# AI4quantum/qiskit-gym

Hardware: AMD Instinct MI355X
Metric: env-steps/sec (whole node), CliffordGym 16q x 65536 envs/GPU; bit-exact vs CPU (higher is better)
Workload: dtype u32

## Files before the change

### qiskit_gym_amd/csrc/kernels_qm_step1.hip

```cpp
#include "device_common.hpp"
#include "qgym_plan.hpp"
#include "qm_step1.hpp"

namespace qg {

constexpr uint32_t QM_STEP1_BLOCK = 256;

template <int NXP, bool HAS_Z, bool FEAT, bool LIST = false, bool DENSE = false>
__global__ __launch_bounds__(QM_STEP1_BLOCK) void qm_step1_kernel(const void *actions, int32_t *depth, uint32_t *bad, const GateEntry *gates, void *state,
                                                                   uint64_t B, uint32_t flags, uint32_t num_actions, StepArgs a) {
    KernelClock kclk(a.kclk, a.kclk_waves, QM_STEP1_BLOCK);
    constexpr int R = HAS_Z ? 2 * NXP : NXP, G = R / 4;
    constexpr int D16 = DENSE ? R / 16 : 0;
    const Step1Front f{actions, depth, bad, gates, state, B, flags, num_actions};
    const uint64_t env = (uint64_t)blockIdx.x * QM_STEP1_BLOCK + threadIdx.x;
    const uint64_t wave_envs = __builtin_amdgcn_ballot_w64(env < B);
    if constexpr (LIST) {
        bool fin = false;
        if (env < B) fin = qm_step1_mask_body<HAS_Z, FEAT, D16>(f, a, G, env, wave_envs);
        done_mask_store(a.done_mask, B, fin, env, a.done_epoch);
    } else {
        if (env >= B) return;
        (void)qm_step1_mask_body<HAS_Z, FEAT, D16>(f, a, G, env, wave_envs);
    }
}

template <int NXP, bool HAS_Z>
static hipError_t launch_step1(const StepArgs &a, hipStream_t s) {
    const dim3 grid((unsigned)((a.B + QM_STEP1_BLOCK - 1) / QM_STEP1_BLOCK)), block(QM_STEP1_BLOCK);
    const bool feat = a.flags & (F_TRACK | F_LAYERS);
    const bool list = a.flags & F_DONE_LIST;
#define QM_STEP1_LAUNCH(...) \
    hipLaunchKernelGGL((qm_step1_kernel<NXP, HAS_Z, __VA_ARGS__>), grid, block, 0, s, a.actions, a.depth, a.bad, a.gates, a.state, a.B, a.flags, a.num_actions, a)
    constexpr int R = HAS_Z ? 2 * NXP : NXP;
    if constexpr (R % 16 == 0) {
        if (a.dense) {
            if (feat && list) QM_STEP1_LAUNCH(true, true, true);
            else if (feat) QM_STEP1_LAUNCH(true, false, true);
            else if (list) QM_STEP1_LAUNCH(false, true, true);
            else QM_STEP1_LAUNCH(false, false, true);
            return hipGetLastError();
        }
    }
    if (feat && list) QM_STEP1_LAUNCH(true, true);
    else if (feat) QM_STEP1_LAUNCH(true);
    else if (list) QM_STEP1_LAUNCH(false, true);
    else QM_STEP1_LAUNCH(false);
#undef QM_STEP1_LAUNCH
    return hipGetLastError();
}

hipError_t qm_step1(const StepArgs &a, uint32_t nxp, bool has_z, hipStream_t s) {
    if (!a.B) return hipSuccess;
    if (has_z) {
        switch (nxp) {
        case 4: return launch_step1<4, true>(a, s);
        case 8: return launch_step1<8, true>(a, s);
        case 12: return launch_step1<12, true>(a, s);
        case 16: return launch_step1<16, true>(a, s);
        }
    } else {
        switch (nxp) {
        case 4: return launch_step1<4, false>(a, s);
        case 8: return launch_step1<8, false>(a, s);
        case 12: return launch_step1<12, false>(a, s);
        case 16: return launch_step1<16, false>(a, s);
        case 20: return launch_step1<20, false>(a, s);
        case 24: return launch_step1<24, false>(a, s);
        case 28: return launch_step1<28, false>(a, s);
        case 32: return launch_step1<32, false>(a, s);
        }
    }
    return hipErrorInvalidValue;
}

}
```

### qiskit_gym_amd/csrc/qgym_api.cpp

```cpp
#include <atomic>
#include <hip/hip_runtime.h>

#include <algorithm>
#include <cmath>
#include <cctype>
#include <cstdarg>
#include <cstdio>
#include <cstdlib>
#include <cstring>
#include <memory>
#include <string>
#include <vector>

#include "pauli_common.hpp"

namespace qg {

static thread_local std::string g_err;

int set_error(int code, const char *fmt, ...) {
    char buf[512];
    va_list ap;
    va_start(ap, fmt);
    vsnprintf(buf, sizeof buf, fmt, ap);
// ... 213 lines not shown
    static const char *one_q[] = {"h", "s", "sdg", "sx", "sxdg"};
    static const char *two_q[] = {"cx", "cz", "swap"};
    for (int k = 0; k < 5; ++k)
        if (key == one_q[k]) {
            if (n != 1) return set_error(QG_ERR_INVALID, "Gate `%s` expects 1 index, got %zu", name.c_str(), n);
            out->kind = k;
            out->q0 = (int32_t)idx[0];
            out->q1 = 0;
            return QG_OK;
        }
    for (int k = 0; k < 3; ++k)
        if (key == two_q[k]) {
            if (n != 2) return set_error(QG_ERR_INVALID, "Gate `%s` expects 2 indices, got %zu", name.c_str(), n);
            out->kind = 5 + k;
            out->q0 = (int32_t)idx[0];
            out->q1 = (int32_t)idx[1];
            return QG_OK;
        }
    return set_error(QG_ERR_INVALID, "Unknown gate name `%s`. Allowed: H, S, Sdg, SX, SXdg, CX, CZ, SWAP", name.c_str());
}


static int vec_free_buffers(qg_vec *v) {
    void *ptrs[] = {v->state, v->own_depth ? v->depth : nullptr, v->own_reward ? v->reward : nullptr,
                    v->own_done ? v->done : nullptr, v->own_success ? v->success : nullptr, v->inverted, v->own_error ? v->error : nullptr, v->sol,
                    v->sol_len, v->layers, v->d_gates, v->d_descs, v->scratch, v->d_prog,
                    v->d_qubit_perms, v->d_act_perms, v->perm_idx, v->d_gen_tables, v->d_nonsymp, v->bad, v->done_list, v->done_list_alt, v->done_list_spare, v->done_mask[0], v->done_mask[1], v->mask_count, v->d_rowops, v->embed_dump, v->host_in, v->host_obs, v->fault_scratch, v->d_twist_obs, v->twist_words};
    for (void *p : ptrs)
        if (p) (void)hipFree(p);
    drop_graphs(v);
    if (v->capture_stream) (void)hipStreamDestroy(v->capture_stream);
    if (v->fault_word) (void)hipHostFree(v->fault_word);
    if (v->count_seen) (void)hipHostFree(v->count_seen);
    return 0;
}

static int drop_done_list(qg_vec *v, hipStream_t s) { return zero_list_length(v, v->done_list, v->dl.drop(), s); }

static void fill_init_args(const qg_vec *v, InitArgs &a) {
    memset(&a, 0, sizeof a);
    a.tree_grid = plan::tree_grid(v->B);
    a.state = v->state;
    a.depth = v->depth;
    a.reward = v->reward;
    a.done = v->done;
    a.success = v->success;
    a.inverted = v->inverted;
    a.error = v->error;
    a.sol_len = v->sol_len;
    a.layers = v->layers;
    a.layers_len = v->layers_len;
    a.gates = v->d_gates;
    a.B = v->B;
    a.D = v->plan.D;
    a.N = v->N;
    a.num_actions = (uint32_t)v->gates.size();
    a.clock = v->clock_dev;
    a.env_base = v->env_base;
    a.bad = v->bad;
    a.rowops = v->d_rowops;
    a.inverts = (v->plan.flags & F_INVERTS) ? 1u : 0u;
    a.check_symplectic = (plan::is_tile(v->plan) && (v->plan.flags & F_INVERTS)) ? 1u : 0u;
}

static hipError_t launch_init(const qg_vec *v, const InitArgs &a_in, hipStream_t s) {
    InitArgs a = a_in;
    a.kclk = kernel_clock_slot(v);
    a.kclk_waves = v->kclk_waves;
    switch (v->plan.layout) {
    case LAYOUT_LFD: return lfd_init(a, v->plan.w64, v->plan.nxp, v->d_descs, s);
    case LAYOUT_LF8: return lf8_init(a, s);
    case LAYOUT_PERM: return perm_init(a, s);
    case LAYOUT_PERMB: return permb_init(a, v->plan.nxp, v->d_descs, s);
    case LAYOUT_TILE: return qm_init(a, v->plan.nxp, v->plan.has_z, s);
    case LAYOUT_TILE64: return q64_init(a, v->plan.nxp, v->plan.has_z, s);
    default: return hipErrorInvalidValue;
    }
}

static hipError_t launch_step(const qg_vec *v, const StepArgs &a_in, hipStream_t s) {
    StepArgs a = a_in;
    a.kclk = kernel_clock_slot(v);
    a.kclk_waves = v->kclk_waves;
    switch (v->plan.layout) {
    case LAYOUT_LFD: return lfd_step(a, v->plan.w64, v->plan.nxp, s);
    case LAYOUT_LF8: return lf8_step(a, a.T > 1, s);
    case LAYOUT_PERM: return perm_step(a, a.T > 1, s);
    case LAYOUT_PERMB: return permb_step(a, v->plan.nxp, s);
    case LAYOUT_PAULI: return pauli_step(v, a, s);
    case LAYOUT_TILE: return qm_step(a, v->plan.nxp, v->plan.has_z, s);
    case LAYOUT_TILE64: return q64_step(a, v->plan.nxp, v->plan.has_z, s);
    default: return hipErrorInvalidValue;
    }
}

static bool dense_rides_in_step(const qg_vec *v) {
    return v->dense && plan::dense_in_kernel(v->plan, plan::step_kernel_of(v->plan, 1, false, false, v->maybe_nonsymplectic, (uint32_t)v->gates.size(), false));
}

int qg_vec_create(const qg_config *cfg, const qg_gate *gates, size_t n_gates, uint64_t batch, int device, qg_vec **out) {
    if (!cfg || !out || (!gates && n_gates)) return set_error(QG_ERR_INVALID, "null argument");
    *out = nullptr;
    if (cfg->num_qubits <= 0) return set_error(QG_ERR_INVALID, "num_qubits must be positive");
    if (cfg->max_depth < 0 || cfg->depth_slope < 0 || cfg->difficulty < 0)
        return set_error(QG_ERR_INVALID, "difficulty, depth_slope and max_depth are usize in the reference");
    if (batch == 0) return set_error(QG_ERR_INVALID, "batch must be positive");
    const uint32_t N = (uint32_t)cfg->num_qubits;
    for (size_t i = 0; i < n_gates; ++i) {
        const qg_gate &g = gates[i];
        if (g.kind < 0 || g.kind > QG_SWAP) return set_error(QG_ERR_INVALID, "gate %zu: unknown kind %d", i, g.kind);
        bool two = g.kind >= QG_CX;
        if (g.q0 < 0 || (uint32_t)g.q0 >= N || (two && (g.q1 < 0 || (uint32_t)g.q1 >= N)))
            return set_error(QG_ERR_INVALID, "gate %zu: qubit index out of range for %u qubits", i, N);
    }

    int ndev = qg_device_count();
    if (ndev <= 0) return set_error(QG_ERR_DEVICE, "no HIP device visible: libqgym has no CPU fallback");
    if (device < 0 || device >= ndev) return set_error(QG_ERR_INVALID, "device %d out of range (%d visible)", device, ndev);
    qg::DeviceGuard guard(device);
    if (guard.err != hipSuccess) {
        (void)hipGetLastError();
        return set_error(QG_ERR_DEVICE, "cannot select device %d: %s", device, hipGetErrorString(guard.err));
    }
    hipDeviceProp_t prop;
    HIP_TRY(hipGetDeviceProperties(&prop, device));
    if (strncmp(prop.gcnArchName, "gfx950", 6) != 0)
        return set_error(QG_ERR_DEVICE, "device %d is %s; libqgym is built for gfx950 (MI355X) only", device, prop.gcnArchName);

    std::unique_ptr<qg_vec> v(new qg_vec());
    v->cfg = *cfg;
    v->gates.assign(gates, gates + n_gates);
    v->B = batch;
    v->N = N;
    v->device = device;
    v->difficulty = cfg->difficulty;
    v->coin_seed = 0x5EED0000C01Full;

    const char *why = "";
    if (int rc = plan::handle_plan(*cfg, batch, v->plan, why)) return set_error(rc, "%s (num_qubits = %u)", why, N);
    const plan::HandlePlan &hp = v->plan;
    if (hp.layout == LAYOUT_PAULI) v->cfg.max_rotations = hp.max_rotations;
    const bool layers = hp.flags & F_LAYERS;

    std::vector<GateEntry> table(std::max<size_t>(n_gates, 1));
    std::vector<uint32_t> descs(std::max<size_t>(n_gates, 1));
    const float w[4] = {cfg->w_n_cnots, cfg->w_n_layers_cnots, cfg->w_n_layers, cfg->w_n_gates};
    for (size_t i = 0; i < n_gates; ++i) {
        int dc, dg;
        gate_deltas(gates[i], N, dc, dg);
        table[i].ops = cfg->env_kind == QG_PAULI ? 0u
                       : hp.layout == LAYOUT_TILE ? tile_ops(cfg->env_kind, gates[i], false)
                       : hp.layout == LAYOUT_TILE64 ? tile_ops(cfg->env_kind, gates[i], true)
                                                  : gate_ops(cfg->env_kind, gates[i], N);
        table[i].penalty = table_penalty(w, dc, dg);
        descs[i] = make_desc((uint32_t)gates[i].kind, (uint32_t)gates[i].q0, (uint32_t)gates[i].q1);
    }

    qg_vec *p = v.get();
    auto fail = [&](int rc) {
        vec_free_buffers(p);
        return rc;
    };
#define HIP_TRY_V(expr)                                                                            \
    do {                                                                                           \
        hipError_t _e = (expr);                                                                    \
        if (_e != hipSuccess) {                                                                    \
// ... 1022 lines not shown
```

### qiskit_gym_amd/csrc/qgym_internal.hpp

```cpp
#pragma once

#include <hip/hip_runtime.h>
#include <stdint.h>

#include "../../include/qgym.h"

namespace qg {

struct GateEntry {
    uint32_t ops;
    float penalty;
};
static_assert(sizeof(GateEntry) == 8, "GateEntry must be 8 bytes");

enum : uint32_t { OP_NONE = 0, OP_XOR = 1, OP_SWAP = 2 };
__host__ __device__ inline uint32_t make_op(uint32_t type, uint32_t dst, uint32_t src) {
    return (dst & 63u) | ((src & 63u) << 6) | ((type & 3u) << 12);
}

__host__ __device__ inline uint32_t make_desc(uint32_t kind, uint32_t q0, uint32_t q1) {
    return (kind & 0xFFu) | ((q0 & 0xFFu) << 8) | ((q1 & 0xFFu) << 16);
}

enum : uint32_t {
    F_ACT64 = 1u << 0,
    F_INVERTS = 1u << 1,
    F_TRACK = 1u << 2,
    F_LAYERS = 1u << 3,
    F_GJ = 1u << 4,
    F_DONE_LIST = 1u << 5,
    F_GROUP_LANES = 1u << 6
};

__host__ __device__ inline uint64_t done_mask_words(uint64_t B) { return 4ull * ((B + 255ull) / 256ull); }
__host__ __device__ inline uint64_t done_mask_bytes(uint64_t B) { return done_mask_words(B) * 10ull + 8ull; }

__host__ __device__ inline uint64_t splitmix64(uint64_t x) {
    x += 0x9E3779B97F4A7C15ull;
    x = (x ^ (x >> 30)) * 0xBF58476D1CE4E5B9ull;
    x = (x ^ (x >> 27)) * 0x94D049BB133111EBull;
    return x ^ (x >> 31);
}
__host__ __device__ inline uint64_t rng_draw(uint64_t seed, uint64_t env, uint64_t t) {
    return splitmix64(seed ^ splitmix64(env * 0x9E3779B97F4A7C15ull + t));
}
__host__ __device__ inline uint32_t rng_action(uint64_t seed, uint64_t env, uint64_t t, uint32_t num_actions) {
#if defined(__HIP_DEVICE_COMPILE__)
    return (uint32_t)__umul64hi(rng_draw(seed, env, t), (uint64_t)num_actions);
#else
    return (uint32_t)(((unsigned __int128)rng_draw(seed, env, t) * (unsigned __int128)num_actions) >> 64);
#endif
}

struct StepArgs {
    void *state;
    const void *actions;
    const uint8_t *coins;
    const GateEntry *gates;
    const uint32_t *descs;
    int32_t *depth;
    float *reward;
    uint8_t *done;
    uint8_t *success;
    uint8_t *inverted;
    uint32_t *error;
    uint32_t *sol;
    int32_t *sol_len;
    int32_t *layers;
    float *rewards_seq;
    uint8_t *dones_seq;
    uint64_t B;
    uint64_t seed;
    uint64_t step_index;
    uint32_t D;
    uint32_t N;
    uint32_t log2L;
    uint32_t num_actions;
    uint32_t T;
    uint32_t flags;
    uint32_t sol_cap;
    float w[4];
    float pauli_layer_reward;
    uint32_t max_rotations;
    uint32_t kclk_waves;
    const uint64_t *clock;
    uint64_t env_base;
    uint32_t *bad;
    unsigned long long *kclk;
    uint32_t *done_list;
    uint32_t *done_count;
    int8_t *dense;
    uint64_t *done_mask;
    uint32_t done_epoch;
};

#if defined(__HIP_DEVICE_COMPILE__) && !defined(QG_NO_ARG_PREFETCH)
#define QG_PREFETCH_STEP_ARGS(a)                                                                                                          \
    asm volatile("" ::"s"((a).state), "s"((a).actions), "s"((a).gates), "s"((a).depth), "s"((a).bad), "s"((a).B), "s"((a).flags),        \
                 "s"((a).num_actions), "s"((a).N), "s"((a).rewards_seq), "s"((a).dones_seq), "s"((a).reward), "s"((a).done), "s"((a).success), \
                 "s"((a).kclk))
#else
#define QG_PREFETCH_STEP_ARGS(a) ((void)0)
#endif

constexpr uint64_t QG_COMPACT_MIN_ENVS = 4096;
constexpr uint64_t QG_STREAM_MIN_ENVS = 64;

struct InitArgs {
    void *state;
    int32_t *depth;
    float *reward;
    uint8_t *done;
    uint8_t *success;
    uint8_t *inverted;
// ... 123 lines not shown
```

### qiskit_gym_amd/csrc/qgym_plan.hpp

```cpp
#pragma once

#include <stdint.h>
#include <stdio.h>

#include "qgym_internal.hpp"

namespace qg {

enum Layout { LAYOUT_NONE = 0, LAYOUT_LF8 = 2, LAYOUT_PERM = 3, LAYOUT_PAULI = 4, LAYOUT_TILE = 5, LAYOUT_TILE64 = 6, LAYOUT_PERMB = 7, LAYOUT_LFD = 8 };

namespace plan {

constexpr uint32_t MAX_PERMUTATION_QUBITS = 256;
constexpr uint32_t MAX_LINEAR_FUNCTION_QUBITS = 64;
constexpr uint32_t MAX_CLIFFORD_QUBITS = 32;
constexpr uint32_t MAX_PAULI_QUBITS = 32;
constexpr uint32_t MAX_PAULI_ROTATIONS = 32;

struct HandlePlan {
    Layout layout = LAYOUT_NONE;
    uint32_t D = 0;
    uint32_t nxp = 0;
    bool has_z = false;
    bool w64 = false;
// ... 74 lines not shown
    if (p.layout == LAYOUT_NONE && p.D <= 32) {
        p.layout = LAYOUT_TILE;
        p.nxp = (N + 3u) & ~3u;
        p.has_z = cfg.env_kind == QG_CLIFFORD;
        p.state_bytes = ((batch + 63) / 64) * (size_t)row_slots(p) * 256;
    }
    if (p.layout == LAYOUT_NONE) {
        p.layout = LAYOUT_TILE64;
        p.has_z = cfg.env_kind == QG_CLIFFORD;
        p.nxp = p.has_z ? 2u * ((N + 3u) & ~3u) : ((N + 7u) & ~7u);
        p.state_bytes = ((batch + 63) / 64) * (size_t)p.nxp * 512;
    }
    if (inverts) p.flags |= F_INVERTS;
    if (cfg.track_solution) p.flags |= F_TRACK;
    if (!(cfg.w_n_layers == 0.0f && cfg.w_n_layers_cnots == 0.0f)) p.flags |= F_LAYERS;
    p.has_bad = (is_tile(p) && !(p.flags & F_INVERTS)) || p.layout == LAYOUT_PERMB || p.layout == LAYOUT_LFD;
    p.has_done_list = is_tile(p) || p.layout == LAYOUT_PAULI;
    if (!p.state_bytes) p.state_bytes = p.stride_bytes * batch;
    return QG_OK;
}

struct CopyRegion {
    uint32_t offset;
    uint32_t rows;
    uint32_t w;
};
constexpr uint32_t COPY_MAX_STATE_REGIONS = 3;
struct CopyLayout {
    CopyRegion r[COPY_MAX_STATE_REGIONS];
    uint32_t n = 0;
    uint32_t tile_bytes = 0;
};
inline CopyLayout copy_layout(const HandlePlan &p) {
    CopyLayout c;
    auto add = [&c](uint32_t rows, uint32_t w) {
        c.r[c.n++] = CopyRegion{c.tile_bytes, rows, w};
        c.tile_bytes += rows * 64u * w;
    };
    switch (p.layout) {
    case LAYOUT_TILE: add(row_slots(p) / 4u, 16); break;
    case LAYOUT_TILE64: add(row_slots(p) / 2u, 16); break;
    case LAYOUT_PERMB: add(p.nxp, 16); break;
    case LAYOUT_LFD: add(2 * p.nxp, 16); break;
    case LAYOUT_LF8:
    case LAYOUT_PERM: add(1, 8); break;
    case LAYOUT_PAULI: {
        const uint32_t meta = p.pt_rm > 16 ? 3u : 1u;
        if (p.pauli_compact) {
            add(p.pt_nq, 12);
            add(p.pt_rm, 8);
            add(meta, 16);
        } else {
            add(p.pt_nq + p.pt_rm + meta, 16);
        }
        break;
    }
    default: break;
    }
    return c;
}
inline void copy_kernel_name(const HandlePlan &p, char *out, size_t cap) {
    const CopyLayout c = copy_layout(p);
    int at = snprintf(out, cap, "copy_envs_kernel [");
    for (uint32_t i = 0; i < c.n && at >= 0 && (size_t)at < cap; ++i)
        at += snprintf(out + at, cap - (size_t)at, "%s%ux%u", i ? " " : "", c.r[i].rows, c.r[i].w);
    if (at >= 0 && (size_t)at < cap) snprintf(out + at, cap - (size_t)at, "]");
}

constexpr uint32_t tile_group_shift(bool has_z) { return has_z ? 1u : 2u; }
constexpr uint32_t GROUP_LANES_MAX_ACTIONS = 256, GROUP_TABLE_DWORDS = 64;
constexpr uint32_t tile_group_byte(uint32_t ops, bool has_z) {
    return ((ops & 31u) >> tile_group_shift(has_z)) | ((((ops >> 5) & 31u) >> tile_group_shift(has_z)) << 4);
}
inline void gate_group_bytes(const uint32_t *ops, size_t stride, size_t num_actions, bool has_z, uint32_t *out) {
    for (uint32_t j = 0; j < GROUP_TABLE_DWORDS; ++j) out[j] = 0;
    for (size_t i = 0; i < num_actions && i < GROUP_LANES_MAX_ACTIONS; ++i) out[i >> 2] |= tile_group_byte(ops[i * stride], has_z) << (8u * (i & 3u));
}

constexpr uint64_t GROUP_LANES_ENVS_PER_WORKGROUP = 256;
constexpr uint64_t GROUP_LANES_WORKGROUPS_PER_CU = 3;
inline bool group_lanes_pays(Layout layout, size_t num_actions, uint64_t batch, uint32_t compute_units) {
    return layout == LAYOUT_TILE && num_actions <= GROUP_LANES_MAX_ACTIONS &&
           batch <= GROUP_LANES_WORKGROUPS_PER_CU * GROUP_LANES_ENVS_PER_WORKGROUP * compute_units;
}

enum StepKernel {
    SK_INVALID = 0,
    SK_QM_STEP1,
    SK_QM_INV2,
    SK_QM_STEP_INV,
    SK_QM_STEP_GJ,
    SK_QM_FUSED_LDS,
    SK_QM_STEP,
    SK_Q64_STEP1, SK_Q64_INV2, SK_Q64_STEP_INV, SK_Q64_STEP_GJ, SK_Q64_FUSED_LDS, SK_Q64_STEP,
    SK_LFD_STEP,
    SK_WORD_STEP,
    SK_PERMB_STEP1, SK_PERMB_STEP,
    SK_PTILE_STEP1C, SK_PTILE_STEP1, SK_PTILE_FUSED1C, SK_PTILE_STEP,
};
inline const char *step_kernel_name(StepKernel k) {
    switch (k) {
    case SK_QM_STEP1: return "qm_step1_kernel";
    case SK_QM_INV2: return "qm_inv2_kernel";
    case SK_QM_STEP_INV: return "qm_step_kernel<inv>";
    case SK_QM_STEP_GJ: return "qm_step_kernel<gauss-jordan>";
    case SK_QM_FUSED_LDS: return "qm_fused_lds_kernel";
    case SK_QM_STEP: return "qm_step_kernel";
    case SK_Q64_STEP1: return "q64_step1_kernel";
    case SK_Q64_INV2: return "q64_inv2_kernel";
    case SK_Q64_STEP_INV: return "q64_step_kernel<inv>";
    case SK_Q64_STEP_GJ: return "q64_step_kernel<gauss-jordan>";
    case SK_Q64_FUSED_LDS: return "q64_fused_lds_kernel";
    case SK_Q64_STEP: return "q64_step_kernel";
    case SK_LFD_STEP: return "lfd_step_kernel";
    case SK_WORD_STEP: return "word_step_kernel";
    case SK_PERMB_STEP1: return "permb_step1_kernel";
    case SK_PERMB_STEP: return "permb_step_kernel";
    case SK_PTILE_STEP1C: return "ptile_step1c_kernel";
    case SK_PTILE_STEP1: return "ptile_step1_kernel";
    case SK_PTILE_FUSED1C: return "ptile_fused1c_kernel";
    case SK_PTILE_STEP: return "ptile_step_kernel";
    default: return "(none)";
    }
}

inline StepKernel tile_step(bool wide, bool inv_kernels, uint32_t flags, uint32_t T, bool has_bad, bool seq_outputs, uint32_t num_actions) {
    const bool feat = flags & (F_TRACK | F_LAYERS);
    const bool seq = T != 1 || seq_outputs;
    if (has_bad && T == 1 && !(flags & F_INVERTS)) return wide ? SK_Q64_STEP1 : SK_QM_STEP1;
    if (flags & F_INVERTS) {
        if (!inv_kernels) return SK_INVALID;
        if (!(flags & F_GJ) && T == 1) return wide ? SK_Q64_INV2 : SK_QM_INV2;
        if (flags & F_GJ) return wide ? SK_Q64_STEP_GJ : SK_QM_STEP_GJ;
        return wide ? SK_Q64_STEP_INV : SK_QM_STEP_INV;
    }
    if (!feat && seq && T > 1 && num_actions != 0) return wide ? SK_Q64_FUSED_LDS : SK_QM_FUSED_LDS;
    return wide ? SK_Q64_STEP : SK_QM_STEP;
}
constexpr bool tile_inv_kernels(bool wide, bool has_z, uint32_t nxp) { return has_z && (wide || nxp <= 16); }
inline StepKernel permb_step_kernel_of(uint32_t flags, uint32_t T, bool has_bad) {
    return (T == 1 && !(flags & F_INVERTS) && has_bad) ? SK_PERMB_STEP1 : SK_PERMB_STEP;
}
inline StepKernel pauli_step_kernel_of(uint32_t flags, uint32_t T, bool compact, bool has_perms) {
    const bool feat = flags & (F_TRACK | F_LAYERS);
    if (T == 1) return compact ? SK_PTILE_STEP1C : SK_PTILE_STEP1;
    if (!feat && !has_perms && compact) return SK_PTILE_FUSED1C;
    return SK_PTILE_STEP;
}
inline StepKernel step_kernel_of(const HandlePlan &p, uint32_t T, bool fused, bool seq_outputs, bool maybe_nonsymplectic, uint32_t num_actions, bool has_perms) {
    const uint32_t flags = p.flags | (maybe_nonsymplectic ? F_GJ : 0u);
    const uint32_t launch_T = fused ? T : 1u;
    switch (p.layout) {
    case LAYOUT_TILE:
    case LAYOUT_TILE64: {
        const bool wide = p.layout == LAYOUT_TILE64;
        return tile_step(wide, tile_inv_kernels(wide, p.has_z, p.nxp), flags, launch_T, p.has_bad, seq_outputs, num_actions);
    }
    case LAYOUT_LFD: return SK_LFD_STEP;
    case LAYOUT_LF8:
    case LAYOUT_PERM: return SK_WORD_STEP;
    case LAYOUT_PERMB: return permb_step_kernel_of(flags, launch_T, p.has_bad);
    case LAYOUT_PAULI: return pauli_step_kernel_of(flags, launch_T, p.pauli_compact, has_perms);
    default: return SK_INVALID;
    }
}
inline bool step_leaves_done_list(const HandlePlan &p, uint64_t batch, bool maybe_nonsymplectic) {
// ... 69 lines not shown
```

### qiskit_gym_amd/csrc/qm_step1.hpp

```cpp
#pragma once

#include "device_common.hpp"

namespace qg {

#define QM_IDENTITY 0x8421u

template <bool HAS_Z>
__device__ inline void qm_group_get(const uint32_t (&u)[4], uint32_t q, uint32_t &x, uint32_t &z) {
    const uint32_t o = 0u - (q & 1u);
    if constexpr (HAS_Z) {
        x = (u[2] & o) | (u[0] & ~o);
        z = (u[3] & o) | (u[1] & ~o);
    } else {
        const uint32_t h = 0u - ((q >> 1) & 1u);
        const uint32_t lo = (u[1] & o) | (u[0] & ~o), hi = (u[3] & o) | (u[2] & ~o);
        x = (hi & h) | (lo & ~h);
        z = 0u;
    }
}
template <bool HAS_Z>
__device__ inline void qm_group_put(uint32_t (&u)[4], uint32_t q, uint32_t x, uint32_t z) {
    if constexpr (HAS_Z) {
        const uint32_t o = 0u - (q & 1u);
// ... 149 lines not shown
    if (layered) lt = layers_begin(layer_rec(a.layers, env, 2 * a.N + 2), a.N, a.descs[act]);
    const uint32_t ops = g.ops, q0 = ops & 31u, q1 = (ops >> 5) & 31u;
    GateMasks<HAS_Z> gm(ops, g0, g1);
    uint32_t e0[4], e1[4];
#pragma unroll
    for (uint32_t k = 0; k < 4; ++k) {
        e0[k] = HAS_Z ? gm.o0 : 0u - (uint32_t)((q0 & 3u) == k);
        e1[k] = HAS_Z ? gm.o1 : 0u - (uint32_t)((q1 & 3u) == k);
    }
    const uint32_t live = 0u - (uint32_t)(((ops >> 10) & 0xFFFFu) != QM_IDENTITY);
    const uint32_t zb = 1u << a.N;
    uint32_t ix0 = 1u << q0, ix1 = 1u << q1, iz0 = zb << q0, iz1 = zb << q1;
    uint32_t set0 = live & 1u, set1 = set0 & (uint32_t)(q0 != q1);
    uint32_t bad_rest = bad0 & ~((set0 << q0) | (set1 << q1));
    r_solved = 1.0f - penalty; r_open = 0.0f - penalty;
    fin_open = (uint32_t)(depth == 0);
    const bool apart = g0 != g1;
    gm.pin();
    if constexpr (!HAS_Z) asm volatile("" : "+v"(e0[0]), "+v"(e0[1]), "+v"(e0[2]), "+v"(e0[3]), "+v"(e1[0]), "+v"(e1[1]), "+v"(e1[2]), "+v"(e1[3]));
    asm volatile("" : "+v"(ix0), "+v"(ix1), "+v"(iz0), "+v"(iz1), "+v"(set0), "+v"(set1), "+v"(bad_rest), "+v"(r_solved), "+v"(r_open),
                      "+v"(depth), "+v"(fin_open));
    __builtin_amdgcn_sched_barrier(0);
    uint32_t z0, z1;
    const uint32_t x0 = gm.get(ua, gm.o0, gm.h0, z0), x1 = gm.get(ub, gm.o1, gm.h1, z1);
    const uint32_t nx0 = gm.mix(0, x0, z0, x1, z1), nx1 = gm.mix(2, x0, z0, x1, z1);
    const uint32_t nz0 = HAS_Z ? gm.mix(1, x0, z0, x1, z1) : 0u, nz1 = HAS_Z ? gm.mix(3, x0, z0, x1, z1) : 0u;
    gate_put<HAS_Z>(ub, e1, nx1, nz1);
    ua.x = bit_select(gm.same, ub.x, ua.x); ua.y = bit_select(gm.same, ub.y, ua.y);
    ua.z = bit_select(gm.same, ub.z, ua.z); ua.w = bit_select(gm.same, ub.w, ua.w);
    gate_put<HAS_Z>(ua, e0, nx0, nz0);
    if (apart) global_store4(pb, ub);
    global_store4(pa, ua);
    if constexpr (D16 > 0) {
        drow[0] = q0; dword[0] = nx0; dchg |= (uint32_t)(nx0 != x0);
        drow[1] = a.N + q0; dword[1] = nz0; dchg |= (uint32_t)(HAS_Z && nz0 != z0) << 1;
        drow[2] = q1; dword[2] = nx1; dchg |= (uint32_t)(q1 != q0 && nx1 != x1) << 2;
        drow[3] = a.N + q1; dword[3] = nz1; dchg |= (uint32_t)(HAS_Z && q1 != q0 && nz1 != z1) << 3;
    }
    const uint32_t d0 = HAS_Z ? xor_or(nx0, ix0, nz0 ^ iz0) : nx0 ^ ix0, d1 = HAS_Z ? xor_or(nx1, ix1, nz1 ^ iz1) : nx1 ^ ix1;
    bad = bad_rest | (min(d0, set0) << q0) | (min(d1, set1) << q1);
    if (layered) {
        penalty = layers_commit(lt, a.w);
        r_solved = 1.0f - penalty; r_open = 0.0f - penalty;
    }
    if constexpr (D16 == 2) {
        const bool solo = (env ^ 1ull) >= f.B;
#pragma unroll
        for (int k = 0; k < 4; ++k) {
            if (solo && ((dchg >> k) & 1u)) dense_row_store<2>(a.dense, env, drow[k], dword[k]);
            const uint32_t mine = (!solo && ((dchg >> k) & 1u)) ? (drow[k] | 0x80000000u) : 0u;
#pragma unroll
            for (int par = 0; par < 2; ++par) {
                const uint32_t r = par ? (uint32_t)__builtin_amdgcn_update_dpp(0, (int)mine, 0xF5, 0xF, 0xF, false)
                                       : (uint32_t)__builtin_amdgcn_update_dpp(0, (int)mine, 0xA0, 0xF, 0xF, false);
                const uint32_t w = par ? (uint32_t)__builtin_amdgcn_update_dpp(0, (int)dword[k], 0xF5, 0xF, 0xF, false)
                                       : (uint32_t)__builtin_amdgcn_update_dpp(0, (int)dword[k], 0xA0, 0xF, 0xF, false);
                const uint64_t e = (env & ~1ull) | (uint64_t)par;
                const uint32_t half = lane & 1u;
                if (r >> 31) *reinterpret_cast<uint4 *>(a.dense + (e * 32u + (r & 31u)) * 32u + 16u * half) = expand16_i8(w >> (16u * half));
            }
        }
    } else if constexpr (D16 == 1) {
#pragma unroll
        for (int k = 0; k < 4; ++k)
            if ((dchg >> k) & 1u) dense_row_store<1>(a.dense, env, drow[k], dword[k]);
    }
    if (FEAT && (f.flags & F_TRACK)) {
        if ((uint32_t)sol_n < a.sol_cap) sol_at(a, env, (uint32_t)sol_n++) = sol_word_framed(act, false);
        else fault |= 8u;
    }
    const bool solved = bad == 0;
    const float reward = solved ? r_solved : r_open;
    const uint32_t fin = solved ? 1u : fin_open;
    if (a.rewards_seq) global_store(out_rseq, reward);
    if (a.dones_seq) global_store(out_dseq, (uint8_t)fin);
    if (bad != bad0) f.bad[env] = bad;
    if (depth != depth0) f.depth[env] = depth;
    global_store(out_reward, reward);
    if (fin != done0) global_store(out_done, (uint8_t)fin);
    if ((uint32_t)solved != success0) global_store(out_success, (uint8_t)solved);
    if (FEAT && (f.flags & F_TRACK)) a.sol_len[env * 2] = sol_n;
    if (FEAT && fault) atomicOr(&a.error[env], fault);
    return fin != 0;
}

template <bool HAS_Z, bool FEAT, int D16, bool PINNED_FRONT>
__device__ inline bool qm_step1_plain_body(const Step1Front &f, const StepArgs &a, uint32_t G, uint64_t env, int64_t act, bool alone) {
    const uint32_t lane = (uint32_t)env & (QG_WAVE - 1);
    uint4 *tile = reinterpret_cast<uint4 *>(f.state) + (env >> 6) * (uint64_t)(G * 64);
    int32_t depth, sol_n;
    uint32_t bad0;
    bool in_range;
    GateEntry g = GateEntry{QM_IDENTITY << 10, 0.0f};
    if constexpr (PINNED_FRONT) {
        int32_t act_lo = 0, act_hi = 0;
        action_issue(f.actions, env, f.flags & F_ACT64, act_lo, act_hi);
        depth = f.depth[env];
        bad0 = f.bad[env];
        sol_n = (FEAT && (f.flags & F_TRACK)) ? a.sol_len[env * 2] : 0;
        __builtin_amdgcn_sched_barrier(0);
        act = action_value(act_lo, act_hi, f.flags & F_ACT64);
        in_range = (uint64_t)act < (uint64_t)f.num_actions;
        const GateEntry entry = f.gates[in_range ? act : 0];
        if (in_range) g = entry;
        asm volatile("" : "+v"(g.ops), "+v"(g.penalty), "+v"(depth), "+v"(bad0)
                     : "s"(a.N), "s"(a.rewards_seq), "s"(a.dones_seq), "s"(a.reward), "s"(a.done), "s"(a.success));
        depth = depth > 0 ? depth - 1 : 0;
    } else {
        depth = f.depth[env];
        bad0 = f.bad[env];
        sol_n = (FEAT && (f.flags & F_TRACK)) ? a.sol_len[env * 2] : 0;
        in_range = act >= 0 && act < (int64_t)f.num_actions;
        if (in_range) g = f.gates[act];
    }
    uint32_t bad = bad0, fault = 0;
    float penalty = 0.0f;
    uint32_t drow[4] = {0, 0, 0, 0}, dword[4] = {0, 0, 0, 0}, dchg = 0;
    if (in_range) {
        penalty = g.penalty;
        const bool layered = FEAT && (f.flags & F_LAYERS);
        LayerTxn lt;
        if (layered) lt = layers_begin(layer_rec(a.layers, env, 2 * a.N + 2), a.N, a.descs[act]);
        const uint32_t q0 = g.ops & 31u, q1 = (g.ops >> 5) & 31u, m = (g.ops >> 10) & 0xFFFFu;
        if (m != QM_IDENTITY) {
            constexpr uint32_t gsh = HAS_Z ? 1u : 2u;
            const uint32_t g0 = q0 >> gsh, g1 = q1 >> gsh;
            const uint4 va = tile[g0 * 64 + lane], vb = tile[g1 * 64 + lane];
            uint32_t ua[4] = {va.x, va.y, va.z, va.w}, ub[4] = {vb.x, vb.y, vb.z, vb.w};
            uint32_t x0, z0, x1, z1;
            qm_group_get<HAS_Z>(ua, q0, x0, z0);
            qm_group_get<HAS_Z>(ub, q1, x1, z1);
            auto mix = [&](uint32_t k) -> uint32_t {
                const uint32_t b = m >> (4 * k);
                uint32_t o = ((0u - (b & 1u)) & x0) ^ ((0u - ((b >> 2) & 1u)) & x1);
                if (HAS_Z) o ^= ((0u - ((b >> 1) & 1u)) & z0) ^ ((0u - ((b >> 3) & 1u)) & z1);
                return o;
            };
            const uint32_t nx0 = mix(0), nx1 = mix(2), nz0 = HAS_Z ? mix(1) : 0u, nz1 = HAS_Z ? mix(3) : 0u;
            qm_group_put<HAS_Z>(ub, q1, nx1, nz1);
            const bool same = g0 == g1;
#pragma unroll
            for (int k = 0; k < 4; ++k) ua[k] = same ? ub[k] : ua[k];
            qm_group_put<HAS_Z>(ua, q0, nx0, nz0);
            if (!same) tile[g1 * 64 + lane] = make_uint4(ub[0], ub[1], ub[2], ub[3]);
            tile[g0 * 64 + lane] = make_uint4(ua[0], ua[1], ua[2], ua[3]);
            if constexpr (D16 > 0) {
                drow[0] = q0; dword[0] = nx0; dchg |= (uint32_t)(nx0 != x0);
                drow[1] = a.N + q0; dword[1] = nz0; dchg |= (uint32_t)(HAS_Z && nz0 != z0) << 1;
                drow[2] = q1; dword[2] = nx1; dchg |= (uint32_t)(q1 != q0 && nx1 != x1) << 2;
                drow[3] = a.N + q1; dword[3] = nz1; dchg |= (uint32_t)(HAS_Z && q1 != q0 && nz1 != z1) << 3;
            }
            const uint32_t zb = 1u << a.N;
            const uint32_t b1 = (uint32_t)(nx1 != (1u << q1) || (HAS_Z && nz1 != (zb << q1)));
            const uint32_t b0 = (uint32_t)(nx0 != (1u << q0) || (HAS_Z && nz0 != (zb << q0)));
            bad = (bad & ~(1u << q1)) | (b1 << q1);
            bad = (bad & ~(1u << q0)) | (b0 << q0);
        }
        if (layered) penalty = layers_commit(lt, a.w);
    }
    if constexpr (D16 == 2) {
        const bool solo = alone || (env ^ 1ull) >= f.B;
#pragma unroll
        for (int k = 0; k < 4; ++k) {
            if (solo && ((dchg >> k) & 1u)) dense_row_store<2>(a.dense, env, drow[k], dword[k]);
            const uint32_t mine = (!solo && ((dchg >> k) & 1u)) ? (drow[k] | 0x80000000u) : 0u;
#pragma unroll
// ... 41 lines not shown
```

Before: 25.65 billion.

## Add straight-line specialized step1 kernel for plain tile layout single steps

Adds a specialized single-step kernel for the tile layout that runs when no tracking, inverts, done-list, dense, sequence outputs or clock are requested. It uses 32-bit byte offsets, reads the gate group table through a wave permute, and places the loads and compute in a hand-ordered sequence held by scheduling barriers and register pins. The goal is to shorten per-env address arithmetic and instruction latency on the hot path. The cost is a separate code path that must stay bit-exact with the general kernel, and it only applies when the batch is a multiple of 64 and within the group-lanes size limit.

```diff
diff --git a/qiskit_gym_amd/csrc/kernels_qm_step1.hip b/qiskit_gym_amd/csrc/kernels_qm_step1.hip
--- a/qiskit_gym_amd/csrc/kernels_qm_step1.hip
+++ b/qiskit_gym_amd/csrc/kernels_qm_step1.hip
@@ -26,10 +26,25 @@
 }
 
 template <int NXP, bool HAS_Z>
+__global__ __launch_bounds__(QM_STEP1_BLOCK) void qm_step1_straight_kernel(const void *actions, int32_t *depth, uint32_t *bad, const GateEntry *gates, void *state,
+                                                                            uint64_t B, uint32_t flags, uint32_t num_actions, StepArgs a) {
+    constexpr int R = HAS_Z ? 2 * NXP : NXP, G = R / 4;
+    const Step1Front f{actions, depth, bad, gates, state, B, flags, num_actions};
+    const uint32_t env = blockIdx.x * QM_STEP1_BLOCK + threadIdx.x;
+    if (env >= (uint32_t)B) return;
+    qm_step1_straight_body<HAS_Z>(f, a, G, env);
+}
+
+template <int NXP, bool HAS_Z>
 static hipError_t launch_step1(const StepArgs &a, hipStream_t s) {
     const dim3 grid((unsigned)((a.B + QM_STEP1_BLOCK - 1) / QM_STEP1_BLOCK)), block(QM_STEP1_BLOCK);
     const bool feat = a.flags & (F_TRACK | F_LAYERS);
     const bool list = a.flags & F_DONE_LIST;
+    if (a.flags & F_STEP1_STRAIGHT) {
+        if (feat || list || a.dense || a.rewards_seq || a.dones_seq || a.kclk || (a.flags & F_ACT64) || a.B % 64u) return hipErrorInvalidValue;
+        hipLaunchKernelGGL((qm_step1_straight_kernel<NXP, HAS_Z>), grid, block, 0, s, a.actions, a.depth, a.bad, a.gates, a.state, a.B, a.flags, a.num_actions, a);
+        return hipGetLastError();
+    }
 #define QM_STEP1_LAUNCH(...) \
     hipLaunchKernelGGL((qm_step1_kernel<NXP, HAS_Z, __VA_ARGS__>), grid, block, 0, s, a.actions, a.depth, a.bad, a.gates, a.state, a.B, a.flags, a.num_actions, a)
     constexpr int R = HAS_Z ? 2 * NXP : NXP;
diff --git a/qiskit_gym_amd/csrc/qgym_api.cpp b/qiskit_gym_amd/csrc/qgym_api.cpp
--- a/qiskit_gym_amd/csrc/qgym_api.cpp
+++ b/qiskit_gym_amd/csrc/qgym_api.cpp
@@ -319,6 +319,9 @@
     StepArgs a = a_in;
     a.kclk = kernel_clock_slot(v);
     a.kclk_waves = v->kclk_waves;
+    if (a.T == 1 && a.bad && plan::step1_straight(v->plan.layout, a.flags, a.num_actions, a.B, device_compute_units(v->device),
+                                                  a.rewards_seq || a.dones_seq, v->kclk != nullptr, a.dense != nullptr))
+        a.flags |= F_STEP1_STRAIGHT;
     switch (v->plan.layout) {
     case LAYOUT_LFD: return lfd_step(a, v->plan.w64, v->plan.nxp, s);
     case LAYOUT_LF8: return lf8_step(a, a.T > 1, s);
diff --git a/qiskit_gym_amd/csrc/qgym_internal.hpp b/qiskit_gym_amd/csrc/qgym_internal.hpp
--- a/qiskit_gym_amd/csrc/qgym_internal.hpp
+++ b/qiskit_gym_amd/csrc/qgym_internal.hpp
@@ -29,7 +29,8 @@
     F_LAYERS = 1u << 3,
     F_GJ = 1u << 4,
     F_DONE_LIST = 1u << 5,
-    F_GROUP_LANES = 1u << 6
+    F_GROUP_LANES = 1u << 6,
+    F_STEP1_STRAIGHT = 1u << 7
 };
 
 __host__ __device__ inline uint64_t done_mask_words(uint64_t B) { return 4ull * ((B + 255ull) / 256ull); }
diff --git a/qiskit_gym_amd/csrc/qgym_plan.hpp b/qiskit_gym_amd/csrc/qgym_plan.hpp
--- a/qiskit_gym_amd/csrc/qgym_plan.hpp
+++ b/qiskit_gym_amd/csrc/qgym_plan.hpp
@@ -180,6 +180,14 @@
 inline bool group_lanes_pays(Layout layout, size_t num_actions, uint64_t batch, uint32_t compute_units) {
     return layout == LAYOUT_TILE && num_actions <= GROUP_LANES_MAX_ACTIONS &&
            batch <= GROUP_LANES_WORKGROUPS_PER_CU * GROUP_LANES_ENVS_PER_WORKGROUP * compute_units;
+}
+
+constexpr uint64_t STEP1_STRAIGHT_MAX_ENVS = 1ull << 24;
+inline bool step1_straight(Layout layout, uint32_t flags, size_t num_actions, uint64_t batch, uint32_t compute_units, bool seq_outputs, bool clock_attached,
+                           bool dense) {
+    return layout == LAYOUT_TILE && !(flags & (F_ACT64 | F_INVERTS | F_TRACK | F_LAYERS | F_DONE_LIST)) && !dense && batch % 64u == 0 &&
+           batch <= STEP1_STRAIGHT_MAX_ENVS && num_actions <= GROUP_LANES_MAX_ACTIONS && group_lanes_pays(layout, num_actions, batch, compute_units) &&
+           !seq_outputs && !clock_attached;
 }
 
 enum StepKernel {
diff --git a/qiskit_gym_amd/csrc/qm_step1.hpp b/qiskit_gym_amd/csrc/qm_step1.hpp
--- a/qiskit_gym_amd/csrc/qm_step1.hpp
+++ b/qiskit_gym_amd/csrc/qm_step1.hpp
@@ -255,6 +255,92 @@
     if (FEAT && (f.flags & F_TRACK)) a.sol_len[env * 2] = sol_n;
     if (FEAT && fault) atomicOr(&a.error[env], fault);
     return fin != 0;
+}
+
+typedef uint32_t u32x2 __attribute__((ext_vector_type(2)));
+template <class T>
+__device__ inline T lane_load(const void *base, uint32_t byte_off) { return *(global_ptr<const T>)((global_ptr<const char>)base + byte_off); }
+template <class T>
+__device__ inline void lane_store(void *base, uint32_t byte_off, T v) {
+    asm volatile("" : "+v"(byte_off));
+    *(global_ptr<T>)((global_ptr<char>)base + byte_off) = v;
+}
+
+template <bool HAS_Z>
+__device__ inline void qm_step1_straight_body(const Step1Front &f, const StepArgs &a, uint32_t G, uint32_t env) {
+    const uint32_t at4 = env << 2;
+    const int32_t act = lane_load<int32_t>(f.actions, at4);
+    __builtin_amdgcn_sched_barrier(0);
+    const uint32_t lane = env & (QG_WAVE - 1);
+    uint32_t at_tile = (env >> 6) * (G * 1024u) + (lane << 4);
+    const uint32_t gtab = lane_load<uint32_t>(f.gates + f.num_actions, lane << 2);
+    int32_t depth0 = lane_load<int32_t>(f.depth, at4);
+    uint32_t bad0 = lane_load<uint32_t>(f.bad, at4);
+    __builtin_amdgcn_sched_barrier(0);
+    uint32_t done0 = lane_load<uint8_t>(a.done, env), success0 = lane_load<uint8_t>(a.success, env);
+    asm volatile("" : "+v"(at_tile));
+    asm volatile("" : : "s"(a.N), "s"(a.reward));
+    __builtin_amdgcn_sched_barrier(0);
+    const uint32_t gi = min((uint32_t)act, f.num_actions);
+    const u32x2 entry = lane_load<u32x2>(f.gates, gi << 3);
+    __builtin_amdgcn_sched_barrier(0);
+    uint32_t gb = (uint32_t)__builtin_amdgcn_ds_bpermute((int)(gi & ~3u), (int)gtab);
+    const bool in_range = (uint32_t)act < f.num_actions;
+    gb = in_range ? gb : 0u;
+    const uint32_t sh = (gi << 3) & 24u;
+    const uint32_t g0 = __builtin_amdgcn_ubfe(gb, sh, 4u), g1 = __builtin_amdgcn_ubfe(gb, sh + 4u, 4u);
+    const uint32_t at_a = at_tile + (g0 << 10), at_b = at_tile + (g1 << 10);
+    const u32x4 va = lane_load<u32x4>(f.state, at_a), vb = lane_load<u32x4>(f.state, at_b);
+    uint4 ua = make_uint4(va.x, va.y, va.z, va.w), ub = make_uint4(vb.x, vb.y, vb.z, vb.w);
+    __builtin_amdgcn_sched_barrier(0);
+    uint32_t g_ops = in_range ? entry.x : QM_IDENTITY << 10;
+    float g_penalty = in_range ? __uint_as_float(entry.y) : 0.0f;
+    asm volatile("" : "+v"(g_ops), "+v"(g_penalty), "+v"(depth0), "+v"(bad0) : "s"(a.N), "s"(a.reward), "s"(a.done), "s"(a.success));
+    asm volatile("" : "+v"(done0), "+v"(success0));
+    int32_t depth = depth0 > 0 ? depth0 - 1 : 0;
+    float r_solved = 0.0f, r_open = 0.0f;
+    uint32_t fin_open = 0;
+    const uint32_t ops = g_ops, q0 = ops & 31u, q1 = (ops >> 5) & 31u;
+    GateMasks<HAS_Z> gm(ops, g0, g1);
+    uint32_t e0[4], e1[4];
+#pragma unroll
+    for (uint32_t k = 0; k < 4; ++k) {
+        e0[k] = HAS_Z ? gm.o0 : 0u - (uint32_t)((q0 & 3u) == k);
+        e1[k] = HAS_Z ? gm.o1 : 0u - (uint32_t)((q1 & 3u) == k);
+    }
+    const uint32_t live = 0u - (uint32_t)(((ops >> 10) & 0xFFFFu) != QM_IDENTITY);
+    const uint32_t zb = 1u << a.N;
+    uint32_t ix0 = 1u << q0, ix1 = 1u << q1, iz0 = zb << q0, iz1 = zb << q1;
+    uint32_t set0 = live & 1u, set1 = set0 & (uint32_t)(q0 != q1);
+    uint32_t bad_rest = bad0 & ~((set0 << q0) | (set1 << q1));
+    r_solved = 1.0f - g_penalty; r_open = 0.0f - g_penalty;
+    fin_open = (uint32_t)(depth == 0);
+    const bool apart = g0 != g1;
+    gm.pin();
+    if constexpr (!HAS_Z) asm volatile("" : "+v"(e0[0]), "+v"(e0[1]), "+v"(e0[2]), "+v"(e0[3]), "+v"(e1[0]), "+v"(e1[1]), "+v"(e1[2]), "+v"(e1[3]));
+    asm volatile("" : "+v"(ix0), "+v"(ix1), "+v"(iz0), "+v"(iz1), "+v"(set0), "+v"(set1), "+v"(bad_rest), "+v"(r_solved), "+v"(r_open),
+                      "+v"(depth), "+v"(fin_open));
+    __builtin_amdgcn_sched_barrier(0);
+    uint32_t z0, z1;
+    const uint32_t x0 = gm.get(ua, gm.o0, gm.h0, z0), x1 = gm.get(ub, gm.o1, gm.h1, z1);
+    const uint32_t nx0 = gm.mix(0, x0, z0, x1, z1), nx1 = gm.mix(2, x0, z0, x1, z1);
+    const uint32_t nz0 = HAS_Z ? gm.mix(1, x0, z0, x1, z1) : 0u, nz1 = HAS_Z ? gm.mix(3, x0, z0, x1, z1) : 0u;
+    gate_put<HAS_Z>(ub, e1, nx1, nz1);
+    ua.x = bit_select(gm.same, ub.x, ua.x); ua.y = bit_select(gm.same, ub.y, ua.y);
+    ua.z = bit_select(gm.same, ub.z, ua.z); ua.w = bit_select(gm.same, ub.w, ua.w);
+    gate_put<HAS_Z>(ua, e0, nx0, nz0);
+    if (apart) lane_store(f.state, at_b, u32x4{ub.x, ub.y, ub.z, ub.w});
+    lane_store(f.state, at_a, u32x4{ua.x, ua.y, ua.z, ua.w});
+    const uint32_t d0 = HAS_Z ? xor_or(nx0, ix0, nz0 ^ iz0) : nx0 ^ ix0, d1 = HAS_Z ? xor_or(nx1, ix1, nz1 ^ iz1) : nx1 ^ ix1;
+    const uint32_t bad = bad_rest | (min(d0, set0) << q0) | (min(d1, set1) << q1);
+    const bool solved = bad == 0;
+    const float reward = solved ? r_solved : r_open;
+    const uint32_t fin = solved ? 1u : fin_open;
+    if (bad != bad0) lane_store(f.bad, at4, bad);
+    if (depth != depth0) lane_store(f.depth, at4, depth);
+    lane_store(a.reward, at4, reward);
+    if (fin != done0) lane_store(a.done, env, (uint8_t)fin);
+    if ((uint32_t)solved != success0) lane_store(a.success, env, (uint8_t)solved);
 }
 
 template <bool HAS_Z, bool FEAT, int D16, bool PINNED_FRONT>
```

Result: faster. 26.10 billion (median of 6 runs) (+1.8%).
